# latteine1217/NSFnet

Measured on AMD Instinct MI355X. Metric: collocation-pt NS-residual evals/sec, Re=2000 6x256 MLP, higher is better.
Workload: dtype bf16x3 (bf16 MFMA, hi/lo split, f32 accumulate)

## Files before the change

nsfnet_amd/csrc/capi.hip:

```cpp
#include <cmath>
#include <cstdio>
#include <cstring>
#include <cstdlib>
#include <new>

#include "../../include/nsfnet_pinn.h"
#include "kernels.h"
#include "optim.h"
#include "rwf.h"

static_assert((int)PINN_FLD_COUNT == (int)FLD_COUNT, "field plane enum mismatch");

static thread_local char g_err[512] = "";
static int fail(int code, const char* fmt, const char* a = "", long b = 0) {
  snprintf(g_err, sizeof(g_err), fmt, a, b);
  return code;
}
static int hipfail(int rc, const char* what) {
  if (rc == -1000) return fail(-22, "%s: unsupported hidden width (code %ld)", what, (long)rc);
  return fail(rc, "%s: HIP error %ld", what, (long)-rc);
}

struct Switches {
  int sched_f, sched_b;
  int wsplit, fuse;
  int stagger;
  int s0_skip32;
  int verbose;
  int tile_cols;
};
static int env_int(const char* name, int dflt) {
  const char* v = getenv(name);
  return v ? atoi(v) : dflt;
}
static Switches read_switches() {
  const int sched = env_int("PINN_SCHED", 2);
  return {env_int("PINN_FWD_SCHED", sched), env_int("PINN_BWD_SCHED", sched), env_int("PINN_WSPLIT", 1),
          env_int("PINN_FUSE", 1), env_int("PINN_STAGGER", 0), env_int("PINN_S0_SKIP32", 1),
          env_int("PINN_VERBOSE", 0), env_int("PINN_TILE_COLS", 0)};
}

struct pinn_net_s {
  int n_out, L, H, HP;
  int wide;
  int prec_fwd, prec_bwd, prec_dw;
};
static int terms_of(int prec) { return prec == 1 ? 3 : 1; }
static int pick_wide(const pinn_net_s* n) {
  if (n->HP > 256) return 1;
  if (n->HP != 256 && n->HP != 128) return 0;
  const bool fp32 = !n->prec_fwd && !n->prec_bwd && !n->prec_dw;
  const int force = read_switches().tile_cols;
  if (force == 64) return 1;
  if (force == 128) return 0;
  return fp32 && n->HP == 256;
}

enum Family { FAM_NONE = 0, FAM_FP32, FAM_FP32_WIDE, FAM_BF16, FAM_BF16_WIDE, FAM_PIPE, FAM_SPLIT, FAM_WSPLIT, FAM_FUSED };
static constexpr const char* FAMILY_NAMES[][3] = {
    {nullptr, nullptr, nullptr},
    {"fwd_kernel", "bwd_kernel", "dw_kernel"},
    {"fwd_wide_kernel", "bwd_wide_kernel", "dw_wide_kernel"},
// ... 7 lines not shown
static Family base_family(const pinn_net_s& n, int prec) {
  return prec ? (n.HP > 256 ? FAM_BF16_WIDE : FAM_BF16) : n.wide ? FAM_FP32_WIDE : FAM_FP32;
}

enum { ROLE_FWD_SAVE = 0, ROLE_FWD, ROLE_BWD, ROLE_DW, ROLE_FUSED, ROLE_COUNT };
struct Role {
  Family family;
  int grid;
  size_t lds;
  const char* name;
};

struct SpillFormat {
  int s24w;
  int s0_skip;
  int s0_skip32;
  int sl0; size_t sblk;
};

struct pinn_plan_s {
  pinn_net_s net;
  long n;
  int streams, ntiles, npad;
  int groups;
  int stagger;
  Role role[ROLE_COUNT];
  SpillFormat spill;
  size_t off_partials, off_oadj, off_sg, off_slabs, off_S, off_Zb, bytes_fwd, bytes_all;
};

static int num_cus() {
  int dev = 0, n = 0;
  if (hipGetDevice(&dev) == hipSuccess &&
      hipDeviceGetAttribute(&n, hipDeviceAttributeMultiprocessorCount, dev) == hipSuccess && n > 0)
    return n;
  (void)hipGetLastError();
  return 256;
}

static size_t align_up(size_t v, size_t a) { return (v + a - 1) / a * a; }

static size_t fwd_lds(Family f, const pinn_net_s& n) {
  switch (f) {
    case FAM_FP32: return fwd_lds_bytes(n.HP);
    case FAM_FP32_WIDE: return fwd_wide_lds_bytes(n.HP);
    case FAM_BF16: return fwd_bf16_lds_bytes(n.HP, n.L, n.wide ? 64 : 128);
    case FAM_BF16_WIDE: return fwd_bf16_wide_lds_bytes(n.HP, n.L);
// ... 101 lines not shown
  if (sf == 1 && fwd_lds(FAM_PIPE, net) > PINN_LDS_MAX) sf = 0;
  if (sb == 2 && bwd_lds(FAM_SPLIT, net) > PINN_LDS_MAX) sb = 1;
  if (sb == 1 && bwd_lds(FAM_PIPE, net) > PINN_LDS_MAX) sb = 0;
  if (sf < 0 || sf > 2) sf = 0;
  if (sb < 0 || sb > 2) sb = 0;
  SpillFormat& sp = p->spill;
  sp.s0_skip = sf == 2 && sb == 2 && net.prec_dw;
  if (!sp.s0_skip) { if (sf == 2) sf = 1; if (sb == 2) sb = 1; }
  sp.s24w = HP > 256 && streams == 4 && net.prec_fwd && net.prec_bwd && net.prec_dw;
  const bool wsplit = sp.s24w && L >= 2 && sw.wsplit != 0 && fwd_lds(FAM_WSPLIT, net) <= PINN_LDS_MAX &&
                      bwd_lds(FAM_WSPLIT, net) <= PINN_LDS_MAX;
  const bool fuse = sf == 2 && sb == 2 && sp.s0_skip && net.prec_fwd == net.prec_bwd && sw.fuse != 0 &&
                    fwdbwd_split_lds_bytes(HP, L) <= PINN_LDS_MAX;
  p->stagger = sw.stagger;
  if (sw.verbose)
    fprintf(stderr, "[pinn] plan: %ld pts, %d streams, HP %d, L %d, prec %d/%d/%d, wide %d, schedule fwd %d bwd %d\n",
            (long)n_points, streams, HP, L, net.prec_fwd, net.prec_bwd, net.prec_dw, (int)wide, sf, sb);
  const Family fs = wsplit ? FAM_WSPLIT : sf == 2 ? FAM_SPLIT : sf == 1 ? FAM_PIPE : f8;
  const Family bs = wsplit ? FAM_WSPLIT : sb == 2 ? FAM_SPLIT : sb == 1 ? FAM_PIPE : b8;
  role(ROLE_FWD, f8, grid_f, lds_f, 0);
  role(ROLE_FWD_SAVE, fs, fs == f8 ? grid_f : grid_fp, fwd_lds(fs, net), 0);
  role(ROLE_BWD, bs, bs == b8 ? grid_b : grid_fp, bwd_lds(bs, net), 1);
  role(ROLE_FUSED, fuse ? FAM_FUSED : FAM_NONE, grid_fp, fuse ? fwdbwd_split_lds_bytes(HP, L) : 0, 0);
  if (L > 1) {
    int g = cus * bpc(lds_d) / (L - 1);
    if (g < 1) g = 1;
    if (g > p->ntiles) g = p->ntiles;
    p->groups = g;
  } else {
    p->groups = 0;
  }
  role(ROLE_DW, d8, p->groups, lds_d, 2);
  const int grid_part = p->role[ROLE_FWD].grid > p->role[ROLE_FWD_SAVE].grid ? p->role[ROLE_FWD].grid : p->role[ROLE_FWD_SAVE].grid;
  size_t off = 0;
  p->off_partials = off; off = align_up(off + (size_t)grid_part * PINN_NLOSS * 4, 256);
  p->off_oadj = off;     off = align_up(off + (size_t)4 * p->npad * 4, 256);
  p->bytes_fwd = off;
  p->off_sg = off;       off = align_up(off + (size_t)p->role[ROLE_BWD].grid * sg_total(HP, L) * 4, 256);
  p->off_slabs = off;    off = align_up(off + (size_t)(L - 1) * p->groups * HP * HP * 4, 256);
  const size_t ablk = (size_t)HP * (wide ? 64 : PINN_TILE_COLS);
  sp.s0_skip32 = streams == 4 && L >= 2 && !net.prec_fwd && !net.prec_bwd && !net.prec_dw && sw.s0_skip32 != 0;
  sp.sl0 = sp.s0_skip ? 1 : 0;
  sp.sblk = sp.s0_skip ? ablk / 4 * 3 : 0;
  const size_t spill_tile = sp.s0_skip ? (size_t)(L - 1) * sp.sblk : (size_t)L * ablk;
  p->off_S = off;        off = align_up(off + (size_t)(p->ntiles + 1) * spill_tile * 4, 256);
  p->off_Zb = off;       off = align_up(off + (size_t)(p->ntiles + 1) * spill_tile * 4, 256);
  p->bytes_all = off;
  return 0;
}

static void stamp_spill(FwdArgs& a, const SpillFormat& f) { a.s24 = f.s24w; a.sl0 = f.sl0; a.sblk = f.sblk; a.s0_skip = f.s0_skip32; }
static void stamp_spill(BwdArgs& a, const SpillFormat& f) { a.s24 = f.s24w; a.sl0 = f.sl0; a.sblk = f.sblk; a.s0_skip = f.s0_skip32; }
static void stamp_spill(DwArgs& a, const SpillFormat& f) { a.s24 = f.s24w; a.sl0 = f.sl0; a.sblk = f.sblk; a.s0_skip = f.s0_skip || f.s0_skip32; }

static float* ws_at(void* ws, size_t off) { return ws ? reinterpret_cast<float*>(reinterpret_cast<char*>(ws) + off) : nullptr; }
#define WS(p, off) ws_at(ws, (p)->off)

static FwdArgs fwd_args(const pinn_plan_s* plan, void* ws, const float* prep, const float* x, const float* y, int save, float scale) {
  FwdArgs a;
  memset(&a, 0, sizeof(a));
  a.x = x; a.y = y; a.n = (int)plan->n; a.ntiles = plan->ntiles; a.L = plan->net.L; a.n_out = plan->net.n_out;
  a.prep = prep; a.S = save ? WS(plan, off_S) : nullptr;
// ... 14 lines not shown
static BwdArgs bwd_args(const pinn_plan_s* plan, void* ws, const float* prep, const float* x, const float* y, float scale) {
  BwdArgs a;
  memset(&a, 0, sizeof(a));
  a.x = x; a.y = y; a.n = (int)plan->n; a.ntiles = plan->ntiles; a.L = plan->net.L; a.n_out = plan->net.n_out;
  a.prep = prep; a.S = WS(plan, off_S); a.Zb = WS(plan, off_Zb);
  a.scale = scale;
  a.sg = WS(plan, off_sg);
  stamp_spill(a, plan->spill);
  return a;
}
static BwdArgs residual_bwd_args(const pinn_plan_s* plan, void* ws, const float* prep, const float* x, const float* y,
                                 const float* e, const float* w, const float* vis_t, const float* fields,
                                 const float* coef_eq4, float Re, float coord_scale, float* ebar_out) {
  BwdArgs a = bwd_args(plan, ws, prep, x, y, coord_scale);
  a.fld = fields; a.e = e; a.w = w; a.vis_used = vis_t;
  for (int k = 0; k < 4; ++k) a.coef_eq[k] = coef_eq4[k];
  a.inv_re = 1.0f / Re; a.ebar = ebar_out;
  return a;
}
static DwArgs dw_args(const pinn_plan_s* plan, void* ws, const float* prep, const float* x, const float* y) {
  DwArgs d;
  memset(&d, 0, sizeof(d));
  d.S = WS(plan, off_S); d.Zb = WS(plan, off_Zb);
  d.ntiles = plan->ntiles; d.L = plan->net.L; d.groups = plan->groups;
  d.slabs = WS(plan, off_slabs);
  d.x = x; d.y = y; d.prep = prep; d.n = (int)plan->n;
  stamp_spill(d, plan->spill);
  return d;
}

static int configure_plan(const pinn_plan_s* p) {
  FwdArgs fa = fwd_args(p, nullptr, nullptr, nullptr, nullptr, 0, 1.f);
  BwdArgs ba = bwd_args(p, nullptr, nullptr, nullptr, nullptr, 1.f);
  DwArgs da = dw_args(p, nullptr, nullptr, nullptr, nullptr);
  fa.configure = ba.configure = da.configure = 1;
  int rc = run_fwd(p, p->role[ROLE_FWD], fa, nullptr);
  if (!rc && p->role[ROLE_FWD_SAVE].family != p->role[ROLE_FWD].family) rc = run_fwd(p, p->role[ROLE_FWD_SAVE], fa, nullptr);
  if (!rc) rc = run_bwd(p, ba, nullptr);
  if (!rc && p->role[ROLE_FUSED].family) rc = run_fused(p, fa, ba, nullptr);
  if (!rc) rc = run_dw(p, da, nullptr);
  return rc;
}

extern "C" {

const char* pinn_last_error(void) { return g_err; }
int pinn_abi_version(void) { return 3; }

int pinn_net_create(int n_out, int n_hidden_layers, int hidden, pinn_net_t* out) {
  if (!out) return fail(-22, "pinn_net_create: null out%s");
  if (n_out < 1 || n_out > 3) return fail(-22, "pinn_net_create: n_out must be 1..3%s");
  if (n_hidden_layers < 1 || n_hidden_layers > 64) return fail(-22, "pinn_net_create: hidden layers must be 1..64%s");
  if (hidden < 1 || hidden > PINN_MAX_HP) return fail(-22, "pinn_net_create: hidden width must be 1..512 (got %s%ld)", "", hidden);
  pinn_net_s* n = new (std::nothrow) pinn_net_s;
  if (!n) return fail(-12, "pinn_net_create: out of host memory%s");
  n->n_out = n_out; n->L = n_hidden_layers; n->H = hidden; n->HP = (hidden + 31) / 32 * 32;
  n->prec_fwd = n->prec_bwd = n->prec_dw = 0;
  n->wide = pick_wide(n);
  *out = n;
  return 0;
}
int pinn_net_set_precision(pinn_net_t net, int prec_fwd, int prec_bwd, int prec_dw) {
  if (!net) return fail(-22, "pinn_net_set_precision: null net%s");
  if (prec_fwd < 0 || prec_fwd > 2 || prec_bwd < 0 || prec_bwd > 2 || prec_dw < 0 || prec_dw > 2)
    return fail(-22, "pinn_net_set_precision: precision must be 0 (fp32), 1 (bf16x3) or 2 (bf16)%s");
  net->prec_fwd = prec_fwd; net->prec_bwd = prec_bwd; net->prec_dw = prec_dw;
  net->wide = pick_wide(net);
  return 0;
}
int pinn_net_destroy(pinn_net_t net) { delete net; return 0; }
int64_t pinn_net_num_params(pinn_net_t net) { return net ? (int64_t)flat_total(net->H, net->L, net->n_out) : -1; }
int64_t pinn_net_prep_floats(pinn_net_t net) { return net ? (int64_t)prep_total(net->HP, net->L) : -1; }

int pinn_net_prepare(pinn_net_t net, const float* params, float* prep, void* stream) {
  if (!net || !params || !prep) return fail(-22, "pinn_net_prepare: null argument%s");
// ... 125 lines not shown
  return run_loss_sums(r, a, loss_sums, (hipStream_t)stream, "pinn_value_forward(loss sums)");
}

int pinn_value_backward(pinn_plan_t plan, void* ws, const float* prep,
                        const float* x, const float* y, const float* out_adj, void* stream) {
  if (!plan || !ws || !prep || !x || !y) return fail(-22, "pinn_value_backward: null argument%s");
  if (plan->streams != 1) return fail(-22, "pinn_value_backward: plan is not a value (1-stream) plan%s");
  BwdArgs a = bwd_args(plan, ws, prep, x, y, 1.f);
  a.oadj = out_adj ? out_adj : WS(plan, off_oadj);
  int rc = run_bwd(plan, a, (hipStream_t)stream);
  if (rc) return hipfail(rc, "pinn_value_backward");
  rc = run_dw_and_stash(plan, ws, prep, x, y, (hipStream_t)stream);
  return rc ? hipfail(rc, "pinn_value_backward(dW)") : 0;
}

static int reduce_sources(const char* who, const pinn_net_s* net, int nsrc, const pinn_plan_t* plans, void* const* wss,
                          ReduceSrc* src) {
  for (int k = 0; k < nsrc; ++k) {
    pinn_plan_t p = plans[k];
    void* ws = wss[k];
    if (!p || !ws) return fail(-22, "%s: null plan/workspace", who);
    if (p->net.H != net->H || p->net.L != net->L || p->net.n_out != net->n_out)
      return fail(-22, "%s: plan belongs to a different net", who);
    src[k].slabs = WS(p, off_slabs); src[k].groups = p->groups;
    src[k].sg = WS(p, off_sg); src[k].nwg = p->role[ROLE_BWD].grid;
  }
  return 0;
}

int pinn_grad_reduce(pinn_net_t net, int nsrc, const pinn_plan_t* plans, void* const* wss,
                     float* grads, int accumulate, void* stream) {
  if (!net || !plans || !wss || !grads) return fail(-22, "pinn_grad_reduce: null argument%s");
  if (nsrc < 1 || nsrc > 4) return fail(-22, "pinn_grad_reduce: nsrc must be 1..4%s");
  ReduceArgs r;
  memset(&r, 0, sizeof(r));
  r.nsrc = nsrc; r.H = net->H; r.HP = net->HP; r.L = net->L; r.n_out = net->n_out;
  r.grads = grads; r.accumulate = accumulate;
  if (int rc = reduce_sources("pinn_grad_reduce", net, nsrc, plans, wss, r.src)) return rc;
  int rc = launch_reduce(r, (hipStream_t)stream);
  return rc ? hipfail(rc, "pinn_grad_reduce") : 0;
}

int pinn_adam_step(float* params, const float* grads, float* m, float* v, int64_t n,
                   float lr, float beta1, float beta2, float eps, int64_t step, void* stream) {
  if (!params || !grads || !m || !v) return fail(-22, "pinn_adam_step: null argument%s");
  if (step < 1) return fail(-22, "pinn_adam_step: step must be >= 1%s");
  double bc1 = 1.0 - std::pow((double)beta1, (double)step);
// ... 372 lines not shown
```

nsfnet_amd/csrc/dw.hip:

```cpp
#include "kernels.h"

template <int T> struct DwCfg;
template <> struct DwCfg<1> { static constexpr int TM = 1, TN = 1; };
template <> struct DwCfg<2> { static constexpr int TM = 1, TN = 2; };
template <> struct DwCfg<3> { static constexpr int TM = 1, TN = 3; };
template <> struct DwCfg<4> { static constexpr int TM = 2, TN = 2; };
template <> struct DwCfg<5> { static constexpr int TM = 1, TN = 5; };
template <> struct DwCfg<6> { static constexpr int TM = 2, TN = 3; };
template <> struct DwCfg<7> { static constexpr int TM = 1, TN = 7; };
template <> struct DwCfg<8> { static constexpr int TM = 4, TN = 2; };

template <int HP, int NS>
__global__ __launch_bounds__(HP * 2) void dw_kernel(DwArgs a) {
  constexpr int T = HP / 32;
  constexpr int TM = DwCfg<T>::TM, TN = DwCfg<T>::TN;
  constexpr int WN = T / TN;
  constexpr int LDW = HP + 4;
  constexpr int CH = 32;
  extern __shared__ float lds[];
  float* Zs = lds;
  float* As = lds + 2 * CH * LDW;
  const int tid = threadIdx.x, lane = tid & 63, i32 = lane & 31, h = lane >> 5;
  const int w = __builtin_amdgcn_readfirstlane(tid >> 6);
  const int wr = w / WN, wc = w % WN;
  const int l = blockIdx.y + 1;
  const int g = blockIdx.x;
  const int t0 = (int)((long)g * a.ntiles / a.groups), t1 = (int)((long)(g + 1) * a.ntiles / a.groups);
  const int nch = (t1 - t0) * 4;
  const int p = tid & 7, og = tid >> 3;

  f32x16 acc[TM][TN];
#pragma unroll
  for (int m = 0; m < TM; ++m)
#pragma unroll
    for (int n = 0; n < TN; ++n)
#pragma unroll
      for (int r = 0; r < 16; ++r) acc[m][n][r] = 0.f;

  f32x4 zr[4], sr[4];
  const bool rec = NS == 4 && a.s0_skip && l == 1;
  f32x4 wx4 = {0.f, 0.f, 0.f, 0.f}, wy4 = wx4, b4 = wx4;
  if (rec) {
    const f32x4* w0 = reinterpret_cast<const f32x4*>(a.prep + prep_w0x(HP));
    wx4 = w0[og]; wy4 = w0[HP / 4 + og]; b4 = w0[2 * (HP / 4) + og];
  }
  auto gload = [&](int ch) {
    const int tile = t0 + (ch >> 2), c = ch & 3;
    const f32x4* Zg = reinterpret_cast<const f32x4*>(a.Zb + ((size_t)tile * a.L + l) * act_block(HP)) + 8 * c;
    const f32x4* Sg = reinterpret_cast<const f32x4*>(a.S + ((size_t)tile * a.L + (l - 1)) * act_block(HP)) + 8 * c;
    const unsigned lo_ = (unsigned)(og * 32 + p);
// ... 48 lines not shown
  }
  __syncthreads();
  for (int ch = 0; ch < nch; ++ch) {
    const int buf = ch & 1;
    if (ch + 1 < nch) gload(ch + 1);
    const float* zp = Zs + buf * CH * LDW + h * LDW + 32 * (wr * TM) + i32;
    const float* ap = As + buf * CH * LDW + h * LDW + 32 * (wc * TN) + i32;
#pragma unroll
    for (int ks = 0; ks < CH / 2; ++ks) {
      float av[TM], bv[TN];
#pragma unroll
      for (int m = 0; m < TM; ++m) av[m] = zp[2 * ks * LDW + 32 * m];
#pragma unroll
      for (int n = 0; n < TN; ++n) bv[n] = ap[2 * ks * LDW + 32 * n];
#pragma unroll
      for (int m = 0; m < TM; ++m)
#pragma unroll
        for (int n = 0; n < TN; ++n)
          acc[m][n] = __builtin_amdgcn_mfma_f32_32x32x2f32(av[m], bv[n], acc[m][n], 0, 0, 0);
    }
    if (ch + 1 < nch) lstore(buf ^ 1);
    __syncthreads();
  }
  float* slab = a.slabs + ((size_t)(l - 1) * a.groups + g) * HP * HP;
#pragma unroll
  for (int m = 0; m < TM; ++m)
#pragma unroll
    for (int n = 0; n < TN; ++n)
#pragma unroll
      for (int r = 0; r < 16; ++r) {
        int o = 32 * (wr * TM + m) + mfma_row(r, h);
        int i = 32 * (wc * TN + n) + i32;
        slab[(size_t)o * HP + i] = acc[m][n][r];
      }
}

size_t dw_lds_bytes(int HP) { return (size_t)2 * 2 * 32 * (HP + 4) * sizeof(float); }
int dw_threads(int HP) { return HP * 2; }

template <int HP, int NS>
static int launch_one(const DwArgs& a, hipStream_t s) {
  size_t lds = dw_lds_bytes(HP);
  return launch_or_configure(&dw_kernel<HP, NS>, dim3(a.groups, a.L - 1), dim3(HP * 2), lds, s, a.configure, a);
}

#define DW_CASE(hp)                                                         \
  case hp:                                                                  \
    return NS == 4 ? launch_one<hp, 4>(a, s) : launch_one<hp, 1>(a, s);

int launch_dw(int HP, int NS, const DwArgs& a, hipStream_t s) {
  if (a.L <= 1 || a.groups <= 0) return 0;
  switch (HP) {
    DW_CASE(32) DW_CASE(64) DW_CASE(96) DW_CASE(128)
    DW_CASE(160) DW_CASE(192) DW_CASE(224) DW_CASE(256)
    default: return -1000;
  }
}
```

nsfnet_amd/csrc/dw_bf16.hip:

```cpp
#include "kernels.h"
#include "bf16_util.h"

template <int T> struct DwCfgB;
template <> struct DwCfgB<1> { static constexpr int TM = 1, TN = 1; };
template <> struct DwCfgB<2> { static constexpr int TM = 1, TN = 2; };
template <> struct DwCfgB<3> { static constexpr int TM = 1, TN = 3; };
template <> struct DwCfgB<4> { static constexpr int TM = 2, TN = 2; };
template <> struct DwCfgB<5> { static constexpr int TM = 1, TN = 5; };
template <> struct DwCfgB<6> { static constexpr int TM = 2, TN = 3; };
template <> struct DwCfgB<7> { static constexpr int TM = 1, TN = 7; };
template <> struct DwCfgB<8> { static constexpr int TM = 4, TN = 2; };

template <int HP>
struct DwImg {
  static constexpr int PADB = ((64 - 2 * HP) % 256 + 256) % 256;
  static constexpr int RSB = 2 * HP + PADB;
  static constexpr int CH = 32;
  static constexpr int ARR = CH * RSB;
  static constexpr size_t BYTES = (size_t)2 * 4 * ARR;
};

typedef __attribute__((address_space(3))) unsigned char lds_u8;
__device__ __forceinline__ u32x2 tr_read(const lds_u8* p) {
  typedef __attribute__((address_space(3))) s16x4 lds_s16x4;
  s16x4 v = __builtin_amdgcn_ds_read_tr16_b64_v4i16((lds_s16x4*)(p));
  return __builtin_bit_cast(u32x2, v);
}

template <int HP, int NS, int TERMS, int PPL, bool REC, bool P24>
__device__ __forceinline__ void dw_bf16_body(const DwArgs& a) {
  constexpr int CPT = PPL / 8;
  constexpr size_t ABLK = (size_t)HP * 4 * PPL;
  using DI = DwImg<HP>;
  constexpr int T = HP / 32;
  constexpr int TM = DwCfgB<T>::TM, TN = DwCfgB<T>::TN;
  constexpr int WN = T / TN;
  extern __shared__ __attribute__((aligned(16))) unsigned char ldsb[];
  const int tid = threadIdx.x, lane = tid & 63, i32 = lane & 31, h = lane >> 5;
  const int w = __builtin_amdgcn_readfirstlane(tid >> 6);
  const int wr = w / WN, wc = w % WN;
  const int l = blockIdx.y + 1;
  const int g = blockIdx.x;
  const int t0 = (int)((long)g * a.ntiles / a.groups), t1 = (int)((long)(g + 1) * a.ntiles / a.groups);
  const int nch = (t1 - t0) * CPT;
  const int p = tid & 7, og = tid >> 3;

  f32x16 acc[TM][TN];
#pragma unroll
  for (int m = 0; m < TM; ++m)
#pragma unroll
    for (int n = 0; n < TN; ++n)
#pragma unroll
      for (int r = 0; r < 16; ++r) acc[m][n][r] = 0.f;

  constexpr bool rec = REC;
  f32x4 wx4 = {0.f, 0.f, 0.f, 0.f}, wy4 = wx4, b4 = wx4;
  if (rec) {
    const f32x4* w0 = reinterpret_cast<const f32x4*>(a.prep + prep_w0x(HP));
    wx4 = w0[og]; wy4 = w0[HP / 4 + og]; b4 = w0[2 * (HP / 4) + og];
  }
  f32x4 zrA[4], srA[4];
  struct Raw24 { u32x4 z[3], s[3]; float px, py; };
  Raw24 rawA, rawB;
  auto gload24 = [&](int ch, Raw24& R) {
    const int tile = t0 + ch / CPT, c = ch % CPT;
    const unsigned lo_ = (unsigned)(og * PPL + p);
// ... 152 lines not shown
      lstore_r(1, zrA, srA, rawA);
      __syncthreads();
      mfma_chunk(1);
    }
    __syncthreads();
  } else {
  if (nch > 0) {
    gload(0, zrA, srA);
    lstore(0, zrA, srA);
    if (nch > 1) gload(1, zrA, srA);
  }
  __syncthreads();
  for (int ch = 0; ch + 1 < nch; ++ch) {
    const int buf = ch & 1;
    mfma_chunk(buf);
    lstore(buf ^ 1, zrA, srA);
    gload(ch + 2 < nch ? ch + 2 : nch - 1, zrA, srA);
    interleave();
    __syncthreads();
  }
  if (nch > 0) mfma_chunk((nch - 1) & 1);
  __syncthreads();
  }
  float* slab = a.slabs + ((size_t)(l - 1) * a.groups + g) * HP * HP;
#pragma unroll
  for (int m = 0; m < TM; ++m)
#pragma unroll
    for (int n = 0; n < TN; ++n)
#pragma unroll
      for (int r = 0; r < 16; ++r) {
        int o = 32 * (wr * TM + m) + mfma_row(r, h);
        int i = 32 * (wc * TN + n) + i32;
        slab[(size_t)o * HP + i] = acc[m][n][r];
      }
}

template <int HP, int NS, int TERMS, int PPL, bool P24>
__global__ __launch_bounds__(HP * 2) void dw_bf16_kernel(DwArgs a) {
  if (P24 && blockIdx.y == 0) dw_bf16_body<HP, NS, TERMS, PPL, P24, P24>(a);
  else dw_bf16_body<HP, NS, TERMS, PPL, false, P24>(a);
}

template <int HP>
static size_t lds_bytes_t() { return DwImg<HP>::BYTES; }

size_t dw_bf16_lds_bytes(int HP) {
  switch (HP) {
    case 32: return lds_bytes_t<32>(); case 64: return lds_bytes_t<64>(); case 96: return lds_bytes_t<96>();
    case 128: return lds_bytes_t<128>(); case 160: return lds_bytes_t<160>(); case 192: return lds_bytes_t<192>();
    case 224: return lds_bytes_t<224>(); default: return lds_bytes_t<256>();
  }
}

template <int HP, int NS, int TERMS, int PPL, bool P24 = false>
static int launch_one(const DwArgs& a, hipStream_t s) {
  if (!P24 && HP == 256 && NS == 4 && PPL == 32 && a.s0_skip) return launch_one<HP, NS, TERMS, PPL, HP == 256 && NS == 4 && PPL == 32>(a, s);
  size_t lds = lds_bytes_t<HP>();
  return launch_or_configure(&dw_bf16_kernel<HP, NS, TERMS, PPL, P24>, dim3(a.groups, a.L - 1), dim3(HP * 2), lds, s, a.configure, a);
}

template <int HP, int PPL>
static int launch_hp(int NS, int terms, const DwArgs& a, hipStream_t s) {
  if (terms == 3) return NS == 4 ? launch_one<HP, 4, 3, PPL>(a, s) : launch_one<HP, 1, 3, PPL>(a, s);
  return NS == 4 ? launch_one<HP, 4, 1, PPL>(a, s) : launch_one<HP, 1, 1, PPL>(a, s);
}

int launch_dw_bf16(int HP, int NS, int terms, int cols, const DwArgs& a, hipStream_t s) {
  if (a.L <= 1 || a.groups <= 0) return 0;
  if (cols == 64) {
    switch (HP) {
      case 128: return launch_hp<128, 16>(NS, terms, a, s);
      case 256: return launch_hp<256, 16>(NS, terms, a, s);
      default: return -1000;
    }
  }
  switch (HP) {
    case 32: return launch_hp<32, 32>(NS, terms, a, s);
    case 64: return launch_hp<64, 32>(NS, terms, a, s);
    case 96: return launch_hp<96, 32>(NS, terms, a, s);
    case 128: return launch_hp<128, 32>(NS, terms, a, s);
    case 160: return launch_hp<160, 32>(NS, terms, a, s);
    case 192: return launch_hp<192, 32>(NS, terms, a, s);
    case 224: return launch_hp<224, 32>(NS, terms, a, s);
    case 256: return launch_hp<256, 32>(NS, terms, a, s);
    default: return -1000;
  }
}
```

nsfnet_amd/csrc/dw_bf16_wide.hip:

```cpp
#include "kernels.h"
#include "bf16_util.h"

namespace {
struct DI {
  static constexpr int RSB = 2 * 256 + 64;
  static constexpr int CH = 32;
  static constexpr int ARR = CH * RSB;
  static constexpr size_t BYTES = (size_t)2 * 4 * ARR;
};
typedef __attribute__((address_space(3))) unsigned char lds_u8;
__device__ __forceinline__ u32x2 tr_read(const lds_u8* p) {
  typedef __attribute__((address_space(3))) s16x4 lds_s16x4;
  s16x4 v = __builtin_amdgcn_ds_read_tr16_b64_v4i16((lds_s16x4*)(p));
  return __builtin_bit_cast(u32x2, v);
}
}

template <int NS, int TERMS, bool P24>
__global__ __launch_bounds__(512) void dw_bf16_wide_kernel(DwArgs a, int HP) {
  constexpr int TM = 4, TN = 2, WN = 4, PPL = 16, COLS = 64, CPT = PPL / 8;
  extern __shared__ __attribute__((aligned(16))) unsigned char ldsb[];
  const int tid = threadIdx.x, lane = tid & 63, i32 = lane & 31, h = lane >> 5;
  const int w = __builtin_amdgcn_readfirstlane(tid >> 6);
  const int wr = w / WN, wc = w % WN;
  const int T = HP / 32, nblk = (T + 7) / 8;
  const int bi = blockIdx.z / nblk, bj = blockIdx.z % nblk;
  const int l = blockIdx.y + 1, g = blockIdx.x;
  const int t0 = (int)((long)g * a.ntiles / a.groups), t1 = (int)((long)(g + 1) * a.ntiles / a.groups);
  const int nch = (t1 - t0) * CPT;
  const int p = tid & 7, og = tid >> 3;
  const int ogz = bi * 64 + og, oga = bj * 64 + og;
  const bool vz = ogz < HP / 4, va = oga < HP / 4;
  const size_t blk = (size_t)HP * COLS;
  bool live[TM][TN];
#pragma unroll
  for (int m = 0; m < TM; ++m)
#pragma unroll
    for (int n = 0; n < TN; ++n) live[m][n] = (bi * 8 + wr * TM + m < T) && (bj * 8 + wc * TN + n < T);

  f32x16 acc[TM][TN];
#pragma unroll
  for (int m = 0; m < TM; ++m)
#pragma unroll
    for (int n = 0; n < TN; ++n)
#pragma unroll
      for (int r = 0; r < 16; ++r) acc[m][n][r] = 0.f;

  f32x4 zr[4], sr[4];
  u32x4 zp[3], sp[3];
  auto gload = [&](int ch) {
    const int tile = t0 + ch / CPT, c = ch % CPT;
// ... 86 lines not shown
    }
  };
  if (nch > 0) {
    gload(0);
    lstore(0);
    if (nch > 1) gload(1);
  }
  __syncthreads();
  for (int ch = 0; ch + 1 < nch; ++ch) {
    const int buf = ch & 1;
    mfma_chunk(buf);
    lstore(buf ^ 1);
    gload(ch + 2 < nch ? ch + 2 : nch - 1);
    constexpr int NMF = (DI::CH / 16) * TM * TN * (TERMS == 3 ? 3 : 1);
#pragma unroll
    for (int i = 0; i < NMF; ++i) {
      __builtin_amdgcn_sched_group_barrier(0x008, 1, 0);
      __builtin_amdgcn_sched_group_barrier(0x002, 4, 0);
    }
    __syncthreads();
  }
  if (nch > 0) mfma_chunk((nch - 1) & 1);
  __syncthreads();
  float* slab = a.slabs + ((size_t)(l - 1) * a.groups + g) * HP * HP;
#pragma unroll
  for (int m = 0; m < TM; ++m)
#pragma unroll
    for (int n = 0; n < TN; ++n) {
      if (!live[m][n]) continue;
      const int tr = bi * 8 + wr * TM + m, tc = bj * 8 + wc * TN + n;
#pragma unroll
      for (int r = 0; r < 16; ++r) {
        int o = 32 * tr + mfma_row(r, h);
        int i = 32 * tc + i32;
        slab[(size_t)o * HP + i] = acc[m][n][r];
      }
    }
}

size_t dw_bf16_wide_lds_bytes() { return DI::BYTES; }

template <int NS, int TERMS, bool P24 = false>
static int launch_one(int HP, const DwArgs& a, hipStream_t s) {
  if (!P24 && NS == 4 && a.s24) return launch_one<NS, TERMS, NS == 4>(HP, a, s);
  const int nblk = (HP / 32 + 7) / 8;
  return launch_or_configure(&dw_bf16_wide_kernel<NS, TERMS, P24>, dim3(a.groups, a.L - 1, nblk * nblk), dim3(512), DI::BYTES, s, a.configure, a, HP);
}

int launch_dw_bf16_wide(int HP, int NS, int terms, const DwArgs& a, hipStream_t s) {
  if (a.L <= 1 || a.groups <= 0) return 0;
  if (HP <= 256 || HP > 512 || HP % 32) return -1000;
  if (terms == 3) return NS == 4 ? launch_one<4, 3>(HP, a, s) : launch_one<1, 3>(HP, a, s);
  return NS == 4 ? launch_one<4, 1>(HP, a, s) : launch_one<1, 1>(HP, a, s);
}
```

nsfnet_amd/csrc/dw_wide.hip:

```cpp
#include "kernels.h"

template <int NS>
__global__ __launch_bounds__(512) void dw_wide_kernel(DwArgs a, int HP) {
  constexpr int TM = 4, TN = 2, WN = 4, LDW = 260, CH = 32, PPL = 16, COLS = 64;
  extern __shared__ float lds[];
  float* Zs = lds;
  float* As = lds + 2 * CH * LDW;
  const int tid = threadIdx.x, lane = tid & 63, i32 = lane & 31, h = lane >> 5;
  const int w = __builtin_amdgcn_readfirstlane(tid >> 6);
  const int wr = w / WN, wc = w % WN;
  const int T = HP / 32, nblk = (T + 7) / 8;
  const int bi = blockIdx.z / nblk, bj = blockIdx.z % nblk;
  const int l = blockIdx.y + 1, g = blockIdx.x;
  const int t0 = (int)((long)g * a.ntiles / a.groups), t1 = (int)((long)(g + 1) * a.ntiles / a.groups);
  const int nch = (t1 - t0) * (PPL / 8);
  const int p = tid & 7, og = tid >> 3;
  const int ogz = bi * 64 + og, oga = bj * 64 + og;
  const bool vz = ogz < HP / 4, va = oga < HP / 4;
  const size_t blk = (size_t)HP * COLS;

  f32x16 acc[TM][TN];
#pragma unroll
  for (int m = 0; m < TM; ++m)
#pragma unroll
    for (int n = 0; n < TN; ++n)
#pragma unroll
      for (int r = 0; r < 16; ++r) acc[m][n][r] = 0.f;

  f32x4 zr[4], sr[4];
  const bool rec = NS == 4 && a.s0_skip && l == 1;
  f32x4 wx4 = {0.f, 0.f, 0.f, 0.f}, wy4 = wx4, b4 = wx4;
  if (rec && va) {
    const f32x4* w0 = reinterpret_cast<const f32x4*>(a.prep + prep_w0x(HP));
    wx4 = w0[oga]; wy4 = w0[HP / 4 + oga]; b4 = w0[2 * (HP / 4) + oga];
  }
  auto gload = [&](int ch) {
    const int tile = t0 + ch / (PPL / 8), c = ch % (PPL / 8);
// ... 51 lines not shown
  }
  __syncthreads();
  for (int ch = 0; ch < nch; ++ch) {
    const int buf = ch & 1;
    if (ch + 1 < nch) gload(ch + 1);
    const float* zp = Zs + buf * CH * LDW + h * LDW + 32 * (wr * TM) + i32;
    const float* ap = As + buf * CH * LDW + h * LDW + 32 * (wc * TN) + i32;
#pragma unroll
    for (int ks = 0; ks < CH / 2; ++ks) {
      float av[TM], bv[TN];
#pragma unroll
      for (int m = 0; m < TM; ++m) av[m] = zp[2 * ks * LDW + 32 * m];
#pragma unroll
      for (int n = 0; n < TN; ++n) bv[n] = ap[2 * ks * LDW + 32 * n];
#pragma unroll
      for (int m = 0; m < TM; ++m)
#pragma unroll
        for (int n = 0; n < TN; ++n)
          acc[m][n] = __builtin_amdgcn_mfma_f32_32x32x2f32(av[m], bv[n], acc[m][n], 0, 0, 0);
    }
    if (ch + 1 < nch) lstore(buf ^ 1);
    __syncthreads();
  }
  float* slab = a.slabs + ((size_t)(l - 1) * a.groups + g) * HP * HP;
#pragma unroll
  for (int m = 0; m < TM; ++m)
#pragma unroll
    for (int n = 0; n < TN; ++n) {
      const int tr = bi * 8 + wr * TM + m, tc = bj * 8 + wc * TN + n;
      if (tr >= T || tc >= T) continue;
#pragma unroll
      for (int r = 0; r < 16; ++r) {
        int o = 32 * tr + mfma_row(r, h);
        int i = 32 * tc + i32;
        slab[(size_t)o * HP + i] = acc[m][n][r];
      }
    }
}

size_t dw_wide_lds_bytes() { return (size_t)2 * 2 * 32 * 260 * sizeof(float); }

int launch_dw_wide(int HP, int NS, const DwArgs& a, hipStream_t s) {
  if (a.L <= 1 || a.groups <= 0) return 0;
  const int T = HP / 32, nblk = (T + 7) / 8;
  size_t lds = dw_wide_lds_bytes();
  dim3 grid(a.groups, a.L - 1, nblk * nblk);
  if (a.configure) {
    int rc = launch_or_configure(&dw_wide_kernel<4>, grid, dim3(512), lds, s, 1, a, HP);
    return rc ? rc : launch_or_configure(&dw_wide_kernel<1>, grid, dim3(512), lds, s, 1, a, HP);
  }
  return NS == 4 ? launch_or_configure(&dw_wide_kernel<4>, grid, dim3(512), lds, s, 0, a, HP)
                 : launch_or_configure(&dw_wide_kernel<1>, grid, dim3(512), lds, s, 0, a, HP);
}
```

nsfnet_amd/csrc/kernels.h:

```cpp
#pragma once
#include <hip/hip_runtime.h>
#include "layout.h"

typedef float f32x16 __attribute__((ext_vector_type(16)));
typedef float f32x4 __attribute__((ext_vector_type(4)));

#ifdef __HIPCC__
typedef __attribute__((address_space(1))) f32x4 gf32x4;
__device__ __forceinline__ gf32x4* pin_base(const void* q) {
  const unsigned long long b = (unsigned long long)q;
  const unsigned lo = __builtin_amdgcn_readfirstlane((unsigned)b), hi = __builtin_amdgcn_readfirstlane((unsigned)(b >> 32));
  return (gf32x4*)(((unsigned long long)hi << 32) | lo);
}
template <typename... Params, typename... Args>
static int launch_or_configure(void (*kernel)(Params...), dim3 grid, dim3 block, size_t lds, hipStream_t s, int configure,
                               const Args&... args) {
  if (configure)
    return -(int)hipFuncSetAttribute(reinterpret_cast<const void*>(kernel), hipFuncAttributeMaxDynamicSharedMemorySize, PINN_LDS_MAX);
  hipLaunchKernelGGL(kernel, grid, block, lds, s, args...);
  return -(int)hipGetLastError();
}
#endif

enum { FLD_U = 0, FLD_V, FLD_UX, FLD_UY, FLD_VX, FLD_VY, FLD_EQ1, FLD_EQ2, FLD_EQ3, FLD_EQ4, FLD_P, FLD_COUNT };
// ... 25 lines not shown
};
PINN_HD size_t spill_off(int tile, int l, int L, int sl0, size_t sblk, size_t classic) {
  return sblk ? ((size_t)tile * (L - sl0) + (l > sl0 ? l - sl0 : 0)) * sblk : ((size_t)tile * L + l) * classic;
}

struct BwdArgs {
  const float* x; const float* y;
  int n, ntiles, L, n_out;
  const float* prep;
  const float* S;
  float* Zb;
  const float* fld; const float* e; const float* w; const float* vis_used;
  float coef_eq[4];
  float inv_re, scale;
  float* ebar;
  const float* oadj;
  float* sg;
  int configure;
  int s24;
  int sl0; size_t sblk;
  int s0_skip;
};

struct DwArgs {
  const float* S; const float* Zb;
  int ntiles, L, groups;
  float* slabs;
  int configure;
  int s0_skip;
  int s24;
  const float* x; const float* y; const float* prep; int n;
  int sl0; size_t sblk;
};

struct ReduceSrc { const float* slabs; int groups; const float* sg; int nwg; };
struct ReduceArgs {
  ReduceSrc src[4]; int nsrc;
  int H, HP, L, n_out;
  float* grads; int accumulate;
};

struct ReduceLoc { int sgi; int layer; size_t slab_off; };
__device__ __forceinline__ ReduceLoc reduce_locate(size_t p, int H, int HP, int L, int n_out) {
  ReduceLoc r{-1, -1, 0};
  if (p < (size_t)2 * H) {
    int o = (int)(p / 2), j = (int)(p % 2);
    r.sgi = (j == 0 ? sg_w0x(HP, L) : sg_w0y(HP, L)) + o;
  } else if (p < (size_t)3 * H) {
    r.sgi = sg_db(HP, 0) + (int)(p - 2 * H);
  } else if (p < flat_w(H, L)) {
    size_t rel = p - (size_t)3 * H;
    size_t per = (size_t)H * H + H;
    int l = 1 + (int)(rel / per);
    size_t q = rel % per;
    if (q < (size_t)H * H) { r.layer = l; r.slab_off = (q / H) * HP + (q % H); }
    else r.sgi = sg_db(HP, l) + (int)(q - (size_t)H * H);
  } else {
    size_t q = p - flat_w(H, L);
    if (q < (size_t)n_out * H) r.sgi = sg_wout(HP, L) + (int)(q / H) * HP + (int)(q % H);
    else r.sgi = sg_bout(HP, L) + (int)(q - (size_t)n_out * H);
  }
  return r;
}
__device__ __forceinline__ double reduce_source_add(double s, const ReduceSrc& src, const ReduceLoc& loc, int HP,
                                                    size_t SG, int w) {
  const float* base; size_t stride; int n;
  if (loc.layer >= 0) { base = src.slabs + (size_t)(loc.layer - 1) * src.groups * HP * HP + loc.slab_off; stride = (size_t)HP * HP; n = src.groups; }
  else { base = src.sg + loc.sgi; stride = SG; n = src.nwg; }
  int g = w;
  for (; g + 24 < n; g += 32) {
    float v0 = base[(size_t)g * stride], v1 = base[(size_t)(g + 8) * stride];
    float v2 = base[(size_t)(g + 16) * stride], v3 = base[(size_t)(g + 24) * stride];
    s += (double)v0; s += (double)v1; s += (double)v2; s += (double)v3;
  }
  for (; g < n; g += 8) s += (double)base[(size_t)g * stride];
  return s;
}

struct TermReduceArgs {
  ReduceSrc src[4]; int nsrc[3];
  int H, HP, L, n_out;
  float* out[3]; int acc_mask;
  double* partials;
  double* gram;
};

__device__ __forceinline__ void wave_gram(float r, float b, float s, int lane, double* __restrict__ out) {
  const double dr = r, db = b, ds = s;
  double q[6] = {__dmul_rn(dr, dr), __dmul_rn(db, db), __dmul_rn(ds, ds),
                 __dmul_rn(dr, db), __dmul_rn(dr, ds), __dmul_rn(db, ds)};
// ... 106 lines not shown
```

Measured before the change: 43.03 million.

## Allow per-layer workgroup counts for dW kernels via flattened 1D grid

Replaces the uniform groups-per-layer dW grid with a prefix-sum table of workgroup counts per layer, launched as a 1D grid. Each block locates its layer and group by scanning the table, and the reduction reads slabs using the same offsets. A weighted splitter can give the recompute-heavy first layer a different share, but its default weight is 1.0, so the default allocation stays even. Kernel argument structs grow by a 64-entry int array, and each block runs a small lookup loop.

```diff
diff --git a/nsfnet_amd/csrc/capi.hip b/nsfnet_amd/csrc/capi.hip
--- a/nsfnet_amd/csrc/capi.hip
+++ b/nsfnet_amd/csrc/capi.hip
@@ -28,6 +28,8 @@
   int s0_skip32;
   int verbose;
   int tile_cols;
+  int dw_split;
+  int dw_rec_groups;
 };
 static int env_int(const char* name, int dflt) {
   const char* v = getenv(name);
@@ -37,7 +39,8 @@
   const int sched = env_int("PINN_SCHED", 2);
   return {env_int("PINN_FWD_SCHED", sched), env_int("PINN_BWD_SCHED", sched), env_int("PINN_WSPLIT", 1),
           env_int("PINN_FUSE", 1), env_int("PINN_STAGGER", 0), env_int("PINN_S0_SKIP32", 1),
-          env_int("PINN_VERBOSE", 0), env_int("PINN_TILE_COLS", 0)};
+          env_int("PINN_VERBOSE", 0), env_int("PINN_TILE_COLS", 0), env_int("PINN_DW_SPLIT", 1),
+          env_int("PINN_DW_REC_GROUPS", 0)};
 }
 
 struct pinn_net_s {
@@ -91,7 +94,7 @@
   pinn_net_s net;
   long n;
   int streams, ntiles, npad;
-  int groups;
+  int gp[PINN_MAX_LAYERS];
   int stagger;
   Role role[ROLE_COUNT];
   SpillFormat spill;
@@ -239,22 +242,40 @@
   role(ROLE_FWD_SAVE, fs, fs == f8 ? grid_f : grid_fp, fwd_lds(fs, net), 0);
   role(ROLE_BWD, bs, bs == b8 ? grid_b : grid_fp, bwd_lds(bs, net), 1);
   role(ROLE_FUSED, fuse ? FAM_FUSED : FAM_NONE, grid_fp, fuse ? fwdbwd_split_lds_bytes(HP, L) : 0, 0);
+  memset(p->gp, 0, sizeof(p->gp));
   if (L > 1) {
-    int g = cus * bpc(lds_d) / (L - 1);
-    if (g < 1) g = 1;
-    if (g > p->ntiles) g = p->ntiles;
-    p->groups = g;
-  } else {
-    p->groups = 0;
-  }
-  role(ROLE_DW, d8, p->groups, lds_d, 2);
+    const int nl = L - 1, slots = cus * bpc(lds_d);
+    int even = slots / nl;
+    if (even < 1) even = 1;
+    if (even > p->ntiles) even = p->ntiles;
+    double wt[PINN_MAX_LAYERS];
+    int cnt[PINN_MAX_LAYERS];
+    for (int i = 0; i < nl; ++i) { wt[i] = 1.0; cnt[i] = even; }
+    if (sw.dw_split == 0) {
+    } else if (sw.dw_rec_groups > 0 && nl > 1) {
+      int g1 = sw.dw_rec_groups;
+      if (g1 > slots - (nl - 1)) g1 = slots - (nl - 1);
+      if (g1 > p->ntiles) g1 = p->ntiles;
+      if (g1 < 1) g1 = 1;
+      cnt[0] = g1;
+      dw_split(slots - g1, nl - 1, p->ntiles, wt + 1, cnt + 1);
+    } else {
+      if (sp.s0_skip) wt[0] = DW_REC_COST;
+      dw_split(even * nl, nl, p->ntiles, wt, cnt);
+    }
+    for (int i = 0; i < nl; ++i) p->gp[i + 1] = p->gp[i] + cnt[i];
+  }
+  const int dw_grid = L > 1 ? p->gp[L - 1] : 0;
+  if (sw.verbose && L > 1)
+    fprintf(stderr, "[pinn] dW: %d workgroups, layer 1 %d, layer %d %d\n", dw_grid, p->gp[1], L - 1, dw_grid - p->gp[L - 2]);
+  role(ROLE_DW, d8, dw_grid, lds_d, 2);
   const int grid_part = p->role[ROLE_FWD].grid > p->role[ROLE_FWD_SAVE].grid ? p->role[ROLE_FWD].grid : p->role[ROLE_FWD_SAVE].grid;
   size_t off = 0;
   p->off_partials = off; off = align_up(off + (size_t)grid_part * PINN_NLOSS * 4, 256);
   p->off_oadj = off;     off = align_up(off + (size_t)4 * p->npad * 4, 256);
   p->bytes_fwd = off;
   p->off_sg = off;       off = align_up(off + (size_t)p->role[ROLE_BWD].grid * sg_total(HP, L) * 4, 256);
-  p->off_slabs = off;    off = align_up(off + (size_t)(L - 1) * p->groups * HP * HP * 4, 256);
+  p->off_slabs = off;    off = align_up(off + (size_t)dw_grid * HP * HP * 4, 256);
   const size_t ablk = (size_t)HP * (wide ? 64 : PINN_TILE_COLS);
   sp.s0_skip32 = streams == 4 && L >= 2 && !net.prec_fwd && !net.prec_bwd && !net.prec_dw && sw.s0_skip32 != 0;
   sp.sl0 = sp.s0_skip ? 1 : 0;
@@ -315,7 +336,7 @@
   DwArgs d;
   memset(&d, 0, sizeof(d));
   d.S = WS(plan, off_S); d.Zb = WS(plan, off_Zb);
-  d.ntiles = plan->ntiles; d.L = plan->net.L; d.groups = plan->groups;
+  d.ntiles = plan->ntiles; d.L = plan->net.L; memcpy(d.gp, plan->gp, sizeof(d.gp));
   d.slabs = WS(plan, off_slabs);
   d.x = x; d.y = y; d.prep = prep; d.n = (int)plan->n;
   stamp_spill(d, plan->spill);
@@ -343,7 +364,7 @@
 int pinn_net_create(int n_out, int n_hidden_layers, int hidden, pinn_net_t* out) {
   if (!out) return fail(-22, "pinn_net_create: null out%s");
   if (n_out < 1 || n_out > 3) return fail(-22, "pinn_net_create: n_out must be 1..3%s");
-  if (n_hidden_layers < 1 || n_hidden_layers > 64) return fail(-22, "pinn_net_create: hidden layers must be 1..64%s");
+  if (n_hidden_layers < 1 || n_hidden_layers > PINN_MAX_LAYERS) return fail(-22, "pinn_net_create: hidden layers must be 1..64%s");
   if (hidden < 1 || hidden > PINN_MAX_HP) return fail(-22, "pinn_net_create: hidden width must be 1..512 (got %s%ld)", "", hidden);
   pinn_net_s* n = new (std::nothrow) pinn_net_s;
   if (!n) return fail(-12, "pinn_net_create: out of host memory%s");
@@ -515,7 +536,7 @@
     if (!p || !ws) return fail(-22, "%s: null plan/workspace", who);
     if (p->net.H != net->H || p->net.L != net->L || p->net.n_out != net->n_out)
       return fail(-22, "%s: plan belongs to a different net", who);
-    src[k].slabs = WS(p, off_slabs); src[k].groups = p->groups;
+    src[k].slabs = WS(p, off_slabs); memcpy(src[k].gp, p->gp, sizeof(src[k].gp));
     src[k].sg = WS(p, off_sg); src[k].nwg = p->role[ROLE_BWD].grid;
   }
   return 0;
diff --git a/nsfnet_amd/csrc/dw.hip b/nsfnet_amd/csrc/dw.hip
--- a/nsfnet_amd/csrc/dw.hip
+++ b/nsfnet_amd/csrc/dw.hip
@@ -23,9 +23,9 @@
   const int tid = threadIdx.x, lane = tid & 63, i32 = lane & 31, h = lane >> 5;
   const int w = __builtin_amdgcn_readfirstlane(tid >> 6);
   const int wr = w / WN, wc = w % WN;
-  const int l = blockIdx.y + 1;
-  const int g = blockIdx.x;
-  const int t0 = (int)((long)g * a.ntiles / a.groups), t1 = (int)((long)(g + 1) * a.ntiles / a.groups);
+  const DwWho who = dw_locate(a, blockIdx.x);
+  const int l = who.l, g = who.g;
+  const int t0 = (int)((long)g * a.ntiles / who.groups), t1 = (int)((long)(g + 1) * a.ntiles / who.groups);
   const int nch = (t1 - t0) * 4;
   const int p = tid & 7, og = tid >> 3;
 
@@ -120,7 +120,7 @@
     if (ch + 1 < nch) lstore(buf ^ 1);
     __syncthreads();
   }
-  float* slab = a.slabs + ((size_t)(l - 1) * a.groups + g) * HP * HP;
+  float* slab = a.slabs + (size_t)blockIdx.x * HP * HP;
 #pragma unroll
   for (int m = 0; m < TM; ++m)
 #pragma unroll
@@ -139,7 +139,7 @@
 template <int HP, int NS>
 static int launch_one(const DwArgs& a, hipStream_t s) {
   size_t lds = dw_lds_bytes(HP);
-  return launch_or_configure(&dw_kernel<HP, NS>, dim3(a.groups, a.L - 1), dim3(HP * 2), lds, s, a.configure, a);
+  return launch_or_configure(&dw_kernel<HP, NS>, dim3(a.gp[a.L - 1]), dim3(HP * 2), lds, s, a.configure, a);
 }
 
 #define DW_CASE(hp)                                                         \
@@ -147,7 +147,7 @@
     return NS == 4 ? launch_one<hp, 4>(a, s) : launch_one<hp, 1>(a, s);
 
 int launch_dw(int HP, int NS, const DwArgs& a, hipStream_t s) {
-  if (a.L <= 1 || a.groups <= 0) return 0;
+  if (a.L <= 1 || a.gp[a.L - 1] <= 0) return 0;
   switch (HP) {
     DW_CASE(32) DW_CASE(64) DW_CASE(96) DW_CASE(128)
     DW_CASE(160) DW_CASE(192) DW_CASE(224) DW_CASE(256)
diff --git a/nsfnet_amd/csrc/dw_bf16.hip b/nsfnet_amd/csrc/dw_bf16.hip
--- a/nsfnet_amd/csrc/dw_bf16.hip
+++ b/nsfnet_amd/csrc/dw_bf16.hip
@@ -28,7 +28,7 @@
 }
 
 template <int HP, int NS, int TERMS, int PPL, bool REC, bool P24>
-__device__ __forceinline__ void dw_bf16_body(const DwArgs& a) {
+__device__ __forceinline__ void dw_bf16_body(const DwArgs& a, const DwWho& who) {
   constexpr int CPT = PPL / 8;
   constexpr size_t ABLK = (size_t)HP * 4 * PPL;
   using DI = DwImg<HP>;
@@ -39,9 +39,8 @@
   const int tid = threadIdx.x, lane = tid & 63, i32 = lane & 31, h = lane >> 5;
   const int w = __builtin_amdgcn_readfirstlane(tid >> 6);
   const int wr = w / WN, wc = w % WN;
-  const int l = blockIdx.y + 1;
-  const int g = blockIdx.x;
-  const int t0 = (int)((long)g * a.ntiles / a.groups), t1 = (int)((long)(g + 1) * a.ntiles / a.groups);
+  const int l = who.l, g = who.g;
+  const int t0 = (int)((long)g * a.ntiles / who.groups), t1 = (int)((long)(g + 1) * a.ntiles / who.groups);
   const int nch = (t1 - t0) * CPT;
   const int p = tid & 7, og = tid >> 3;
 
@@ -240,7 +239,7 @@
   if (nch > 0) mfma_chunk((nch - 1) & 1);
   __syncthreads();
   }
-  float* slab = a.slabs + ((size_t)(l - 1) * a.groups + g) * HP * HP;
+  float* slab = a.slabs + (size_t)blockIdx.x * HP * HP;
 #pragma unroll
   for (int m = 0; m < TM; ++m)
 #pragma unroll
@@ -255,8 +254,9 @@
 
 template <int HP, int NS, int TERMS, int PPL, bool P24>
 __global__ __launch_bounds__(HP * 2) void dw_bf16_kernel(DwArgs a) {
-  if (P24 && blockIdx.y == 0) dw_bf16_body<HP, NS, TERMS, PPL, P24, P24>(a);
-  else dw_bf16_body<HP, NS, TERMS, PPL, false, P24>(a);
+  const DwWho who = dw_locate(a, blockIdx.x);
+  if (P24 && who.l == 1) dw_bf16_body<HP, NS, TERMS, PPL, P24, P24>(a, who);
+  else dw_bf16_body<HP, NS, TERMS, PPL, false, P24>(a, who);
 }
 
 template <int HP>
@@ -274,7 +274,7 @@
 static int launch_one(const DwArgs& a, hipStream_t s) {
   if (!P24 && HP == 256 && NS == 4 && PPL == 32 && a.s0_skip) return launch_one<HP, NS, TERMS, PPL, HP == 256 && NS == 4 && PPL == 32>(a, s);
   size_t lds = lds_bytes_t<HP>();
-  return launch_or_configure(&dw_bf16_kernel<HP, NS, TERMS, PPL, P24>, dim3(a.groups, a.L - 1), dim3(HP * 2), lds, s, a.configure, a);
+  return launch_or_configure(&dw_bf16_kernel<HP, NS, TERMS, PPL, P24>, dim3(a.gp[a.L - 1]), dim3(HP * 2), lds, s, a.configure, a);
 }
 
 template <int HP, int PPL>
@@ -284,7 +284,7 @@
 }
 
 int launch_dw_bf16(int HP, int NS, int terms, int cols, const DwArgs& a, hipStream_t s) {
-  if (a.L <= 1 || a.groups <= 0) return 0;
+  if (a.L <= 1 || a.gp[a.L - 1] <= 0) return 0;
   if (cols == 64) {
     switch (HP) {
       case 128: return launch_hp<128, 16>(NS, terms, a, s);
diff --git a/nsfnet_amd/csrc/dw_bf16_wide.hip b/nsfnet_amd/csrc/dw_bf16_wide.hip
--- a/nsfnet_amd/csrc/dw_bf16_wide.hip
+++ b/nsfnet_amd/csrc/dw_bf16_wide.hip
@@ -25,8 +25,9 @@
   const int wr = w / WN, wc = w % WN;
   const int T = HP / 32, nblk = (T + 7) / 8;
   const int bi = blockIdx.z / nblk, bj = blockIdx.z % nblk;
-  const int l = blockIdx.y + 1, g = blockIdx.x;
-  const int t0 = (int)((long)g * a.ntiles / a.groups), t1 = (int)((long)(g + 1) * a.ntiles / a.groups);
+  const DwWho who = dw_locate(a, blockIdx.x);
+  const int l = who.l, g = who.g;
+  const int t0 = (int)((long)g * a.ntiles / who.groups), t1 = (int)((long)(g + 1) * a.ntiles / who.groups);
   const int nch = (t1 - t0) * CPT;
   const int p = tid & 7, og = tid >> 3;
   const int ogz = bi * 64 + og, oga = bj * 64 + og;
@@ -159,7 +160,7 @@
   }
   if (nch > 0) mfma_chunk((nch - 1) & 1);
   __syncthreads();
-  float* slab = a.slabs + ((size_t)(l - 1) * a.groups + g) * HP * HP;
+  float* slab = a.slabs + (size_t)blockIdx.x * HP * HP;
 #pragma unroll
   for (int m = 0; m < TM; ++m)
 #pragma unroll
@@ -181,11 +182,11 @@
 static int launch_one(int HP, const DwArgs& a, hipStream_t s) {
   if (!P24 && NS == 4 && a.s24) return launch_one<NS, TERMS, NS == 4>(HP, a, s);
   const int nblk = (HP / 32 + 7) / 8;
-  return launch_or_configure(&dw_bf16_wide_kernel<NS, TERMS, P24>, dim3(a.groups, a.L - 1, nblk * nblk), dim3(512), DI::BYTES, s, a.configure, a, HP);
+  return launch_or_configure(&dw_bf16_wide_kernel<NS, TERMS, P24>, dim3(a.gp[a.L - 1], 1, nblk * nblk), dim3(512), DI::BYTES, s, a.configure, a, HP);
 }
 
 int launch_dw_bf16_wide(int HP, int NS, int terms, const DwArgs& a, hipStream_t s) {
-  if (a.L <= 1 || a.groups <= 0) return 0;
+  if (a.L <= 1 || a.gp[a.L - 1] <= 0) return 0;
   if (HP <= 256 || HP > 512 || HP % 32) return -1000;
   if (terms == 3) return NS == 4 ? launch_one<4, 3>(HP, a, s) : launch_one<1, 3>(HP, a, s);
   return NS == 4 ? launch_one<4, 1>(HP, a, s) : launch_one<1, 1>(HP, a, s);
diff --git a/nsfnet_amd/csrc/dw_wide.hip b/nsfnet_amd/csrc/dw_wide.hip
--- a/nsfnet_amd/csrc/dw_wide.hip
+++ b/nsfnet_amd/csrc/dw_wide.hip
@@ -11,8 +11,9 @@
   const int wr = w / WN, wc = w % WN;
   const int T = HP / 32, nblk = (T + 7) / 8;
   const int bi = blockIdx.z / nblk, bj = blockIdx.z % nblk;
-  const int l = blockIdx.y + 1, g = blockIdx.x;
-  const int t0 = (int)((long)g * a.ntiles / a.groups), t1 = (int)((long)(g + 1) * a.ntiles / a.groups);
+  const DwWho who = dw_locate(a, blockIdx.x);
+  const int l = who.l, g = who.g;
+  const int t0 = (int)((long)g * a.ntiles / who.groups), t1 = (int)((long)(g + 1) * a.ntiles / who.groups);
   const int nch = (t1 - t0) * (PPL / 8);
   const int p = tid & 7, og = tid >> 3;
   const int ogz = bi * 64 + og, oga = bj * 64 + og;
@@ -110,7 +111,7 @@
     if (ch + 1 < nch) lstore(buf ^ 1);
     __syncthreads();
   }
-  float* slab = a.slabs + ((size_t)(l - 1) * a.groups + g) * HP * HP;
+  float* slab = a.slabs + (size_t)blockIdx.x * HP * HP;
 #pragma unroll
   for (int m = 0; m < TM; ++m)
 #pragma unroll
@@ -129,10 +130,10 @@
 size_t dw_wide_lds_bytes() { return (size_t)2 * 2 * 32 * 260 * sizeof(float); }
 
 int launch_dw_wide(int HP, int NS, const DwArgs& a, hipStream_t s) {
-  if (a.L <= 1 || a.groups <= 0) return 0;
+  if (a.L <= 1 || a.gp[a.L - 1] <= 0) return 0;
   const int T = HP / 32, nblk = (T + 7) / 8;
   size_t lds = dw_wide_lds_bytes();
-  dim3 grid(a.groups, a.L - 1, nblk * nblk);
+  dim3 grid(a.gp[a.L - 1], 1, nblk * nblk);
   if (a.configure) {
     int rc = launch_or_configure(&dw_wide_kernel<4>, grid, dim3(512), lds, s, 1, a, HP);
     return rc ? rc : launch_or_configure(&dw_wide_kernel<1>, grid, dim3(512), lds, s, 1, a, HP);
diff --git a/nsfnet_amd/csrc/kernels.h b/nsfnet_amd/csrc/kernels.h
--- a/nsfnet_amd/csrc/kernels.h
+++ b/nsfnet_amd/csrc/kernels.h
@@ -71,9 +71,38 @@
   int s0_skip;
 };
 
+#define PINN_MAX_LAYERS 64
+
+constexpr double DW_REC_COST = 1.0;
+
+inline void dw_split(int slots, int nl, int ntiles, const double* weight, int* count) {
+  double wsum = 0.0;
+  for (int i = 0; i < nl; ++i) wsum += weight[i];
+  const double unit = slots / wsum;
+  int sum = 0;
+  for (int i = 0; i < nl; ++i) {
+    int c = (int)(weight[i] * unit + 1e-9);
+    count[i] = c < 1 ? 1 : c > ntiles ? ntiles : c;
+    sum += count[i];
+  }
+  while (sum != slots) {
+    const int d = sum < slots ? 1 : -1;
+    int best = -1;
+    double gap = 0.0;
+    for (int i = 0; i < nl; ++i) {
+      if (d > 0 ? count[i] >= ntiles : count[i] <= 1) continue;
+      const double q = d * (weight[i] * unit - count[i]);
+      if (best < 0 || q > gap + 1e-9) { best = i; gap = q; }
+    }
+    if (best < 0) break;
+    count[best] += d; sum += d;
+  }
+}
+
 struct DwArgs {
   const float* S; const float* Zb;
-  int ntiles, L, groups;
+  int ntiles, L;
+  int gp[PINN_MAX_LAYERS];
   float* slabs;
   int configure;
   int s0_skip;
@@ -82,7 +111,16 @@
   int sl0; size_t sblk;
 };
 
-struct ReduceSrc { const float* slabs; int groups; const float* sg; int nwg; };
+#ifdef __HIPCC__
+struct DwWho { int l, g, groups; };
+__device__ __forceinline__ DwWho dw_locate(const DwArgs& a, int b) {
+  int l = 1;
+  while (l < a.L - 1 && b >= a.gp[l]) ++l;
+  return DwWho{l, b - a.gp[l - 1], a.gp[l] - a.gp[l - 1]};
+}
+#endif
+
+struct ReduceSrc { const float* slabs; const float* sg; int nwg; int gp[PINN_MAX_LAYERS]; };
 struct ReduceArgs {
   ReduceSrc src[4]; int nsrc;
   int H, HP, L, n_out;
@@ -114,7 +152,10 @@
 __device__ __forceinline__ double reduce_source_add(double s, const ReduceSrc& src, const ReduceLoc& loc, int HP,
                                                     size_t SG, int w) {
   const float* base; size_t stride; int n;
-  if (loc.layer >= 0) { base = src.slabs + (size_t)(loc.layer - 1) * src.groups * HP * HP + loc.slab_off; stride = (size_t)HP * HP; n = src.groups; }
+  if (loc.layer >= 0) {
+    const int g0 = src.gp[loc.layer - 1];
+    base = src.slabs + (size_t)g0 * HP * HP + loc.slab_off; stride = (size_t)HP * HP; n = src.gp[loc.layer] - g0;
+  }
   else { base = src.sg + loc.sgi; stride = SG; n = src.nwg; }
   int g = w;
   for (; g + 24 < n; g += 32) {
```

New measurement: 43.01 million. No clear change (-0.0%).
